# colinsongf/keyword_spotting

Hardware: AMD Instinct MI355X
Metric: mel-frames/s (real-time 10 ms-hop audio streams sustained = value/100) (higher is better)
Workload: dtype f32

## Files before the change

### keyword_spotting_amd/csrc/gru_device.h

```cpp
#pragma once
#include <type_traits>

#include "kws_internal.h"

namespace kws {

typedef float f32x4 __attribute__((ext_vector_type(4)));

__device__ __forceinline__ f32x4 mfma4(float a, float b, f32x4 c) {
    return __builtin_amdgcn_mfma_f32_16x16x4f32(a, b, c, 0, 0, 0);
}
__device__ __forceinline__ float sigmoid_f(float x) {
    return __builtin_amdgcn_rcpf(1.0f + __expf(-x));
}
__device__ __forceinline__ float tanh_f(float x) {
    return 1.0f - 2.0f * __builtin_amdgcn_rcpf(1.0f + __expf(2.0f * x));
}
#if KWS_RESIDENT_VGPR_FORM
#define KWS_MFMA_A(acc, wa, bv) acc = mfma4(wa, bv, acc)
#else
#define KWS_MFMA_A(acc, wa, bv) \
    asm volatile("v_mfma_f32_16x16x4_f32 %0, %1, %2, %0" : "+v"(acc) : "a"(wa), "v"(bv))
#endif
__device__ __forceinline__ void mfma_fence(f32x4& a, f32x4& b, f32x4& c, f32x4& d) {
    asm volatile("s_nop 15" : "+v"(a), "+v"(b), "+v"(c), "+v"(d));
}
__device__ __forceinline__ void mfma_fence(f32x4& a, f32x4& b) {
    asm volatile("s_nop 15" : "+v"(a), "+v"(b));
}
__device__ __forceinline__ void mfma_prefence(f32x4& a, f32x4& b, f32x4& c, f32x4& d) {
    asm volatile("s_nop 3" : "+v"(a), "+v"(b), "+v"(c), "+v"(d));
}
__device__ __forceinline__ void mfma_prefence(f32x4& a, f32x4& b) {
    asm volatile("s_nop 3" : "+v"(a), "+v"(b));
}
__device__ __forceinline__ f32x4 splat4(float v) { f32x4 r = {v, v, v, v}; return r; }
__device__ __forceinline__ float bitsel(unsigned m, float a, float b) {
    return __uint_as_float((__float_as_uint(a) & m) | (__float_as_uint(b) & ~m));
}
template <int I0, int I1, class F>
__device__ __forceinline__ void static_for(F&& f) {
    if constexpr (I0 < I1) {
        f(std::integral_constant<int, I0>{});
        static_for<I0 + 1, I1>(f);
    }
}
constexpr float kLog2e = 1.4426950408889634f;
typedef float f32x2 __attribute__((ext_vector_type(2)));
__device__ __forceinline__ f32x2 sigmoid2(f32x2 x) {
    const f32x2 t = x * -kLog2e;
    f32x2 e;
    e.x = __builtin_amdgcn_exp2f(t.x);
    e.y = __builtin_amdgcn_exp2f(t.y);
    const f32x2 d = e + 1.0f;
    f32x2 r;
    r.x = __builtin_amdgcn_rcpf(d.x);
    r.y = __builtin_amdgcn_rcpf(d.y);
#ifdef KWS_FAULT_INJECT
    r = r * 1.0078125f;
#endif
    return r;
}
__device__ __forceinline__ f32x2 tanh2(f32x2 x) {
    const f32x2 t = x * (2.0f * kLog2e);
    f32x2 e;
    e.x = __builtin_amdgcn_exp2f(t.x);
    e.y = __builtin_amdgcn_exp2f(t.y);
    const f32x2 d = e + 1.0f;
    f32x2 r;
    r.x = __builtin_amdgcn_rcpf(d.x);
    r.y = __builtin_amdgcn_rcpf(d.y);
    return r * -2.0f + 1.0f;
}
__device__ __forceinline__ f32x4 ld4(const float* p) { return *reinterpret_cast<const f32x4*>(p); }

__device__ __forceinline__ void lds_barrier() {
    asm volatile("s_waitcnt lgkmcnt(0)" ::: "memory");
    __builtin_amdgcn_s_barrier();
    asm volatile("" ::: "memory");
}
constexpr int kRingFrames = 16;
constexpr int xs_stride(int kcx) { return 4 * ((((kcx + 3) / 4) & 1) ? (kcx + 3) / 4 : (kcx + 3) / 4 + 1); }
struct EpilogueLds {
    float* pstage;
    float* lring;
    int* words;
    int* carry;
    int8_t* cwords;
};
constexpr size_t kEpilogueLdsBytes = (4 * 16 * 8 + kRingFrames * 16 * 8) * 4 + kRingFrames * 16 * 4 + 2 * 16 * 4;
__device__ __forceinline__ EpilogueLds epilogue_carve(char* base) {
    EpilogueLds e;
    e.pstage = reinterpret_cast<float*>(base);
    e.lring = e.pstage + 4 * 16 * 8;
    e.words = reinterpret_cast<int*>(e.lring + kRingFrames * 16 * 8);
    e.carry = e.words + kRingFrames * 16;
    e.cwords = nullptr;
    return e;
}

__device__ __forceinline__ void epilogue_fold(const EpilogueLds& e, int t, int lane) {
    if (lane < 32) {
        const int s = lane >> 1, half = lane & 1;
        f32x4 v = *reinterpret_cast<const f32x4*>(e.pstage + (0 * 16 + s) * 8 + 4 * half);
#pragma unroll
        for (int w = 1; w < 4; ++w) v += *reinterpret_cast<const f32x4*>(e.pstage + (w * 16 + s) * 8 + 4 * half);
        *reinterpret_cast<f32x4*>(e.lring + (((t & (kRingFrames - 1)) * 16 + s) * 8 + 4 * half)) = v;
    }
}

struct FoldRegs { f32x4 v[4]; };
__device__ __forceinline__ void epilogue_fold_load(const EpilogueLds& e, int lane, FoldRegs& r) {
    if (lane < 32) {
        const int s = lane >> 1, half = lane & 1;
#pragma unroll
        for (int w = 0; w < 4; ++w) r.v[w] = *reinterpret_cast<const f32x4*>(e.pstage + (w * 16 + s) * 8 + 4 * half);
    }
}
__device__ __forceinline__ void epilogue_fold_store(const EpilogueLds& e, int t, int lane, const FoldRegs& r) {
    if (lane < 32) {
        const int s = lane >> 1, half = lane & 1;
        const f32x4 v = ((r.v[0] + r.v[1]) + r.v[2]) + r.v[3];
        *reinterpret_cast<f32x4*>(e.lring + (((t & (kRingFrames - 1)) * 16 + s) * 8 + 4 * half)) = v;
    }
}

template <bool OPAQUE_LANE = false>
__device__ __forceinline__ void epilogue_flush(const GruLayerParams& p, const EpilogueLds& e, int group, int t0,
                                               int n, int w, int lane, bool final_flush) {
    if constexpr (OPAQUE_LANE) asm volatile("" : "+v"(lane));
    const int f = 4 * w + (lane & 3);
    const int s = lane >> 2;
    const int b = group * kStreamsPerGroup + s;
    const int C = p.C;
    float lg[kMaxClasses];
    {
        const f32x4* row = reinterpret_cast<const f32x4*>(e.lring + (f * 16 + s) * 8);
        const f32x4 lo = row[0], hi = row[1];
#pragma unroll
        for (int c = 0; c < 4; ++c) { lg[c] = lo[c]; lg[4 + c] = hi[c]; }
    }
    if (p.use_relu) {
#pragma unroll
        for (int c = 0; c < kMaxClasses; ++c) {
            lg[c] = fmaxf(lg[c], 0.f);
            if (p.value_clip > 0.f) lg[c] = fminf(lg[c], 20.f);
        }
    }
    float m = lg[0];
#pragma unroll
    for (int c = 1; c < kMaxClasses; ++c) m = (c < C) ? fmaxf(m, lg[c]) : m;
    float pr[kMaxClasses];
    float sum = 0.f;
#pragma unroll
    for (int c = 0; c < kMaxClasses; ++c) {
        pr[c] = (c < C) ? __expf(lg[c] - m) : 0.f;
        sum += pr[c];
    }
    const float inv = __builtin_amdgcn_rcpf(sum);
#pragma unroll
    for (int c = 0; c < kMaxClasses; ++c) pr[c] *= inv;
    int word = -1;
    float best = -1.f;
#pragma unroll
    for (int c = 1; c < kMaxClasses - 1; ++c) {
        if (c < C - 1 && pr[c] > best) { best = pr[c]; word = c - 1; }
    }
    if (!(best > p.decode_thres)) word = -1;
    e.words[f * 16 + s] = word;
    if (e.cwords != nullptr) {
        int ln = lane;
        asm volatile("" : "+v"(ln));
        const int f2 = 4 * w + (ln & 3);
        if (f2 < n) e.cwords[(ln >> 2) * kWinTailWordsStride + t0 + f2] = (int8_t)word;
    }
    const bool mine = b < p.B && f < n;
    const size_t row = (size_t)b * (p.t_stride ? p.t_stride : p.T) + (t0 + f);
    if (mine) {
        if (C == 6) {
            if (p.logits) {
                float2* o = reinterpret_cast<float2*>(p.logits + row * 6);
                o[0] = make_float2(lg[0], lg[1]); o[1] = make_float2(lg[2], lg[3]); o[2] = make_float2(lg[4], lg[5]);
            }
            if (p.softmax) {
                float2* o = reinterpret_cast<float2*>(p.softmax + row * 6);
                o[0] = make_float2(pr[0], pr[1]); o[1] = make_float2(pr[2], pr[3]); o[2] = make_float2(pr[4], pr[5]);
            }
        } else {
            if (p.logits) {
#pragma unroll
                for (int c = 0; c < kMaxClasses; ++c)
                    if (c < C) p.logits[row * C + c] = lg[c];
            }
            if (p.softmax) {
#pragma unroll
                for (int c = 0; c < kMaxClasses; ++c)
                    if (c < C) p.softmax[row * C + c] = pr[c];
            }
        }
    }
    lds_barrier();
    const int blk = (t0 / kRingFrames) & 1;
    const int prev = f == 0 ? e.carry[blk * 16 + s] : e.words[(f - 1) * 16 + s];
    const int token = (word >= 0 && word != prev) ? word + 1 : 0;
    if (f == n - 1) {
        if (!final_flush) e.carry[(blk ^ 1) * 16 + s] = word;
        else if (b < p.B && p.prev_word) p.prev_word[b] = word;
    }
    if (mine && p.tokens) p.tokens[row] = (int8_t)token;
}


}
```

### keyword_spotting_amd/csrc/gru_resident.hip

```cpp
#include <cstddef>

#include "gru_device.h"
#include "launch.h"
#include "window_device.h"

namespace kws {

#if KWS_RESIDENT_VGPR_FORM
template <class... A> __device__ __forceinline__ void resident_prefence(A&...) {}
template <class... A> __device__ __forceinline__ void resident_fence(A&...) { __builtin_amdgcn_sched_barrier(0); }
#else
template <class... A> __device__ __forceinline__ void resident_prefence(A&... a) { mfma_prefence(a...); }
template <class... A> __device__ __forceinline__ void resident_fence(A&... a) { mfma_fence(a...); }
#endif


#if KWS_RESIDENT_VGPR_FORM
constexpr int resident_kreg(int kcx, bool first, bool last, bool window) { return first ? kcx : (last && window) ? 10 : 16; }
#else
constexpr int resident_kreg(int, bool first, bool, bool) { return first ? 0 : 2; }
#endif
constexpr size_t resident_lds_bytes(int kcx, bool first, bool last, bool window) {
    size_t n = 2 * 8 * 64 * 16 + (size_t)4 * (kcx - resident_kreg(kcx, first, last, window)) * 64 * 16;
    if (!first) n += 8 * 64 * 16;
    if (last) n += kEpilogueLdsBytes;
    if (first) n += (size_t)64 * xs_stride(kcx) * 4;
    return n;
}

template <int KCX, bool FIRST, bool LAST, bool MASKED, bool WINDOW>
__device__ __forceinline__ void gru_layer_resident_body(const GruLayerParams& p) {
    static_assert(!WINDOW || (LAST && !FIRST), "the window tail belongs to the last layer of a stack");
    static_assert(!WINDOW || !MASKED, "the window tail refuses seq_len");
    constexpr int H = 128, NT = 8, KCH = 32;
    const int tid = threadIdx.x;
    const int w = __builtin_amdgcn_readfirstlane(tid >> 6);
    const int lane = tid & 63, g = lane >> 4, s = lane & 15;
    const int n_groups = (p.B + kStreamsPerGroup - 1) / kStreamsPerGroup;
    int group = blockIdx.x;
    int b_raw = group * kStreamsPerGroup + s;
    bool bvalid = b_raw < p.B;
    int b = bvalid ? b_raw : p.B - 1;
    const int T = p.T;
    const int n0 = 2 * w, n1 = 2 * w + 1;

    extern __shared__ __attribute__((aligned(16))) char smem[];
    f32x4* hbuf = reinterpret_cast<f32x4*>(smem);
    f32x4* rhbuf = hbuf + NT * 64;
    constexpr int KREG = resident_kreg(KCX, FIRST, LAST, WINDOW), KL = KCX - KREG;
    static_assert(KREG >= 0 && KREG <= KCX && 192 + 4 * KREG <= 256, "the register chunks share the 256 AGPRs with the recurrent weights");
    f32x4* wlds = rhbuf + NT * 64;
    f32x4* xsb = wlds + 4 * KL * 64;
    char* const lds_tail = reinterpret_cast<char*>(xsb + (FIRST ? 0 : NT * 64));
    static_assert(resident_lds_bytes(KCX, FIRST, LAST, WINDOW) + (WINDOW ? kWinTailWordsBytes : 0) <= 160 * 1024, "LDS per CU");
    EpilogueLds epi = epilogue_carve(lds_tail);
    if constexpr (WINDOW) epi.cwords = reinterpret_cast<int8_t*>(lds_tail + kEpilogueLdsBytes);
    const uint8_t* win_dl = reinterpret_cast<const uint8_t*>(epi.cwords) + 16 * kWinTailWordsStride;
    constexpr size_t kWinOffset = offsetof(GruLayerParams, win);
    if constexpr (WINDOW) window_tail_prepare(window_tail_params_from_kernarg(kWinOffset), const_cast<uint8_t*>(win_dl), tid);
    constexpr int kXsStride = xs_stride(KCX);
    float* xs = reinterpret_cast<float*>(lds_tail + (LAST ? kEpilogueLdsBytes : 0));

    float wgh[2][2][KCH];
    float wch[2][KCH];
    float wcx[2][KCX];
    float wgx[KREG ? KREG : 1][4];
    const f32x4* wh4 = reinterpret_cast<const f32x4*>(p.wh);
#pragma unroll
    for (int j = 0; j < 2; ++j) {
        const int n = 2 * w + j;
#pragma unroll
        for (int k4 = 0; k4 < KCH / 4; ++k4) {
            const f32x4 vr = wh4[((n * 3 + 0) * (KCH / 4) + k4) * 64 + lane];
            const f32x4 vu = wh4[((n * 3 + 1) * (KCH / 4) + k4) * 64 + lane];
            const f32x4 vc = wh4[((n * 3 + 2) * (KCH / 4) + k4) * 64 + lane];
#pragma unroll
            for (int e = 0; e < 4; ++e) {
                wgh[j][0][4 * k4 + e] = vr[e];
                wgh[j][1][4 * k4 + e] = vu[e];
                wch[j][4 * k4 + e] = vc[e];
            }
        }
    }
    if constexpr (FIRST) {
#pragma unroll
        for (int j = 0; j < 2; ++j)
#pragma unroll
            for (int kc = 0; kc < KCX; ++kc) wcx[j][kc] = p.wx[(((2 * w + j) * 3 + 2) * KCX + kc) * 64 + lane];
#pragma unroll
        for (int kc = 0; kc < KCX; ++kc) {
            f32x4 v;
            v.x = p.wx[((n0 * 3 + 0) * KCX + kc) * 64 + lane];
            v.y = p.wx[((n0 * 3 + 1) * KCX + kc) * 64 + lane];
            v.z = p.wx[((n1 * 3 + 0) * KCX + kc) * 64 + lane];
            v.w = p.wx[((n1 * 3 + 1) * KCX + kc) * 64 + lane];
            if (kc < KREG) { const int kr = kc < KREG ? kc : 0; wgx[kr][0] = v[0]; wgx[kr][1] = v[1]; wgx[kr][2] = v[2]; wgx[kr][3] = v[3]; }
            else wlds[(w * KL + kc - KREG) * 64 + lane] = v;
        }
    } else {
        const f32x4* wx4 = reinterpret_cast<const f32x4*>(p.wx);
#pragma unroll
        for (int j = 0; j < 2; ++j)
#pragma unroll
            for (int k4 = 0; k4 < KCX / 4; ++k4) {
                const f32x4 vc = wx4[(((2 * w + j) * 3 + 2) * (KCX / 4) + k4) * 64 + lane];
#pragma unroll
                for (int e = 0; e < 4; ++e) wcx[j][4 * k4 + e] = vc[e];
            }
#pragma unroll
        for (int k4 = 0; k4 < KCX / 4; ++k4) {
            const f32x4 r0 = wx4[((n0 * 3 + 0) * (KCX / 4) + k4) * 64 + lane];
            const f32x4 u0 = wx4[((n0 * 3 + 1) * (KCX / 4) + k4) * 64 + lane];
            const f32x4 r1 = wx4[((n1 * 3 + 0) * (KCX / 4) + k4) * 64 + lane];
            const f32x4 u1 = wx4[((n1 * 3 + 1) * (KCX / 4) + k4) * 64 + lane];
#pragma unroll
            for (int e = 0; e < 4; ++e) {
                const f32x4 v = {r0[e], u0[e], r1[e], u1[e]};
                const int kc = 4 * k4 + e, kr = kc < KREG ? kc : 0;
                if (kc < KREG) { wgx[kr][0] = v[0]; wgx[kr][1] = v[1]; wgx[kr][2] = v[2]; wgx[kr][3] = v[3]; }
                else wlds[(w * KL + kc - KREG) * 64 + lane] = v;
            }
        }
    }
#pragma unroll
    for (int j = 0; j < 2; ++j) {
#pragma unroll
        for (int kc = 0; kc < KCH; ++kc) {
            asm volatile("" : "+a"(wgh[j][0][kc]));
            asm volatile("" : "+a"(wgh[j][1][kc]));
            asm volatile("" : "+a"(wch[j][kc]));
        }
    }
#if KWS_RESIDENT_VGPR_FORM
    if constexpr (KREG > 0) {
#pragma unroll
        for (int kc = 0; kc < KREG; ++kc)
#pragma unroll
            for (int e = 0; e < 4; ++e) asm volatile("" : "+a"(wgx[kc][e]));
    }
#endif
    asm volatile("s_nop 7" ::: "memory");
    f32x4 bias_r[2], bias_u[2], bias_c[2];
#pragma unroll
    for (int j = 0; j < 2; ++j) {
        const int n = 2 * w + j;
        bias_r[j] = ld4(p.bias + 0 * H + n * 16 + 4 * g);
        bias_u[j] = ld4(p.bias + 1 * H + n * 16 + 4 * g);
        bias_c[j] = ld4(p.bias + 2 * H + n * 16 + 4 * g);
    }
    float wfc[2][4];
    f32x4 bfc4 = splat4(0.f);
    if (LAST) {
#pragma unroll
        for (int j = 0; j < 2; ++j)
#pragma unroll
            for (int e = 0; e < 4; ++e) wfc[j][e] = p.wfc[((2 * w + j) * 4 + e) * 64 + lane];
        if (w == 0) bfc4 = ld4(p.bfc + 4 * g);
    }

    int len_s = T;
    f32x4 hreg[2];
    const float4* xl_src = nullptr;
    const float4* xprev = nullptr;
    const float4* xg_next = nullptr;
    constexpr int XQ = KCX;
    const int xl_row = lane / XQ, xl_q = lane % XQ;
    const bool xl_active = FIRST && lane < 4 * XQ;
    auto enter_group = [&]() {
        b_raw = group * kStreamsPerGroup + s;
        bvalid = b_raw < p.B;
        b = bvalid ? b_raw : p.B - 1;
        const bool do_reset = p.reset != nullptr && p.reset[b] != 0;
        if constexpr (MASKED) len_s = p.seq_len ? p.seq_len[b] - p.t_base : T;
#pragma unroll
        for (int j = 0; j < 2; ++j) {
            const int n = 2 * w + j;
            hreg[j] = do_reset ? splat4(0.f) : ld4(p.state_in + (size_t)b * H + n * 16 + 4 * g);
            hbuf[n * 64 + lane] = hreg[j];
        }
        if (LAST && tid < 16) {
            const int bb = group * kStreamsPerGroup + tid;
            int pw = -1;
            if (bb < p.B && p.prev_word && !(p.reset && p.reset[bb])) pw = p.prev_word[bb];
            epi.carry[tid] = pw;
        }
        if constexpr (FIRST) {
            const int xl_b = min(group * kStreamsPerGroup + 4 * w + (xl_active ? xl_row : 0), p.B - 1);
            xl_src = reinterpret_cast<const float4*>(p.x_mel + (size_t)xl_b * (p.t_stride ? p.t_stride : T) * p.I) + xl_q;
        } else {
            xprev = p.x_prev + (size_t)group * T * NT * 64 + lane;
            xg_next = xprev + ((size_t)(1 < T ? 1 : 0) * NT + n0) * 64;
        }
    };

    constexpr bool kIssueAtEnd = FIRST && !LAST;
    float4 xl_inflight = make_float4(0.f, 0.f, 0.f, 0.f);
    auto coop_issue = [&](int t_req) {
        const int t = t_req < T ? t_req : T - 1;
        if (xl_active) xl_inflight = xl_src[(size_t)t * XQ];
    };
    auto coop_commit = [&]() {
        if (xl_active) {
            float* dst = xs + (4 * (4 * w + xl_row)) * kXsStride + xl_q;
            dst[0 * kXsStride] = xl_inflight.x;
            dst[1 * kXsStride] = xl_inflight.y;
            dst[2 * kXsStride] = xl_inflight.z;
            dst[3 * kXsStride] = xl_inflight.w;
        }
    };
    float xbuf0[KCX];
    auto read_xs = [&](float (&dst)[KCX]) {
        const float* row = xs + (4 * s + g) * kXsStride;
#pragma unroll
        for (int k4 = 0; k4 < KCX / 4; ++k4) {
            const f32x4 v = *reinterpret_cast<const f32x4*>(row + 4 * k4);
            dst[4 * k4 + 0] = v[0]; dst[4 * k4 + 1] = v[1]; dst[4 * k4 + 2] = v[2]; dst[4 * k4 + 3] = v[3];
        }
        if constexpr (KCX % 4 >= 2) {
            const f32x2 v = *reinterpret_cast<const f32x2*>(row + (KCX / 4) * 4);
            dst[(KCX / 4) * 4 + 0] = v[0]; dst[(KCX / 4) * 4 + 1] = v[1];
        }
        if constexpr (KCX % 2 == 1) dst[KCX - 1] = row[KCX - 1];
    };
    auto load_x_slice = [&](float (&dst)[KCX], int t_req, const int sl) {
        if constexpr (!FIRST) {
            const int t = t_req < T ? t_req : T - 1;
            const float4 v = xprev[((size_t)t * NT + sl) * 64];
            dst[4 * sl + 0] = v.x; dst[4 * sl + 1] = v.y; dst[4 * sl + 2] = v.z; dst[4 * sl + 3] = v.w;
        }
    };
    float4 xg_inflight[2];
    auto group_issue = [&](int t_req) {
        if constexpr (!FIRST) {
            xg_inflight[0] = xg_next[0];
            xg_inflight[1] = xg_next[64];
            if (t_req + 1 < T) xg_next += NT * 64;
        }
    };
    auto group_commit = [&]() {
        if constexpr (!FIRST) {
#pragma unroll
            for (int j = 0; j < 2; ++j)
                xsb[(2 * w + j) * 64 + lane] = (f32x4){xg_inflight[j].x, xg_inflight[j].y, xg_inflight[j].z, xg_inflight[j].w};
        }
    };
    auto read_x_slice = [&](float (&dst)[KCX], const int sl) {
        if constexpr (!FIRST) {
            const f32x4 v = xsb[sl * 64 + lane];
            dst[4 * sl + 0] = v[0]; dst[4 * sl + 1] = v[1]; dst[4 * sl + 2] = v[2]; dst[4 * sl + 3] = v[3];
        }
    };

    f32x4 acc_r[2], acc_u[2], acc_c[2];
    auto gates_x_part = [&](const float (&xB)[KCX], auto k0_, auto k1_, auto pin_) {
        constexpr int K0 = decltype(k0_)::value, K1 = decltype(k1_)::value;
        constexpr bool PIN = decltype(pin_)::value;
        constexpr int R0 = K0 < KREG ? KREG : K0;
        f32x4 ring[3];
        if (R0 < K1) ring[R0 % 3] = wlds[(w * KL + R0 - KREG) * 64 + lane];
        if (R0 + 1 < K1) ring[(R0 + 1) % 3] = wlds[(w * KL + R0 + 1 - KREG) * 64 + lane];
#pragma unroll
        for (int kc = K0; kc < K1; ++kc) {
            if (kc + 2 < K1 && kc + 2 >= R0 + 2) ring[(kc + 2) % 3] = wlds[(w * KL + kc + 2 - KREG) * 64 + lane];
            if (PIN) __builtin_amdgcn_sched_barrier(0);
            const int kr = kc < KREG ? kc : 0;
            const f32x4 a4 = kc < KREG ? (f32x4){wgx[kr][0], wgx[kr][1], wgx[kr][2], wgx[kr][3]} : ring[kc % 3];
            acc_r[0] = mfma4(a4.x, xB[kc], acc_r[0]);
            acc_u[0] = mfma4(a4.y, xB[kc], acc_u[0]);
            acc_r[1] = mfma4(a4.z, xB[kc], acc_r[1]);
            acc_u[1] = mfma4(a4.w, xB[kc], acc_u[1]);
            if (PIN) __builtin_amdgcn_sched_barrier(0);
        }
    };
    using pinned = std::true_type;
    constexpr int KSPLIT = KCX / 2;
    using k_lo = std::integral_constant<int, 0>;
    using k_mid = std::integral_constant<int, KSPLIT>;
    using k_hi = std::integral_constant<int, KCX>;
    auto cand_x = [&](const float (&xB)[KCX]) {
#pragma unroll
        for (int j = 0; j < 2; ++j) acc_c[j] = bias_c[j];
#pragma unroll
        for (int kc = 0; kc < KCX; ++kc) {
            acc_c[0] = mfma4(wcx[0][kc], xB[kc], acc_c[0]);
            acc_c[1] = mfma4(wcx[1][kc], xB[kc], acc_c[1]);
        }
    };

    f32x4 hb_a, hb_b;

    auto frame = [&](int t, float (&xcur)[KCX], float (&xnxt)[KCX]) {
        resident_prefence(acc_r[0], acc_u[0], acc_r[1], acc_u[1]);
#pragma unroll
        for (int nn = 0; nn < NT; ++nn) {
            const f32x4 hb = (nn & 1) ? hb_b : hb_a;
            if (nn + 2 < NT) {
                if (nn & 1) hb_b = hbuf[(nn + 2) * 64 + lane]; else hb_a = hbuf[(nn + 2) * 64 + lane];
            }
            if constexpr (FIRST) { if (!kIssueAtEnd && nn == 0) coop_issue(t + 2); }
            else { if (nn == 0) group_issue(t + 2); read_x_slice(xnxt, nn); }
            __builtin_amdgcn_sched_barrier(0);
#pragma unroll
            for (int e = 0; e < 4; ++e) {
                const int kc = 4 * nn + e;
                const float hv = hb[e];
                KWS_MFMA_A(acc_r[0], wgh[0][0][kc], hv);
                KWS_MFMA_A(acc_u[0], wgh[0][1][kc], hv);
                KWS_MFMA_A(acc_r[1], wgh[1][0][kc], hv);
                KWS_MFMA_A(acc_u[1], wgh[1][1][kc], hv);
            }
        }
        resident_fence(acc_r[0], acc_u[0], acc_r[1], acc_u[1]);
        if constexpr (FIRST) read_xs(xcur);
        f32x4 u[2];
#pragma unroll
        for (int j = 0; j < 2; ++j) {
            const f32x2 r_lo = sigmoid2((f32x2){acc_r[j][0], acc_r[j][1]});
            const f32x2 r_hi = sigmoid2((f32x2){acc_r[j][2], acc_r[j][3]});
            const f32x2 rh_lo = r_lo * (f32x2){hreg[j][0], hreg[j][1]};
            const f32x2 rh_hi = r_hi * (f32x2){hreg[j][2], hreg[j][3]};
            rhbuf[(2 * w + j) * 64 + lane] = (f32x4){rh_lo.x, rh_lo.y, rh_hi.x, rh_hi.y};
        }
#pragma unroll
        for (int j = 0; j < 2; ++j) {
            const f32x2 u_lo = sigmoid2((f32x2){acc_u[j][0], acc_u[j][1]});
            const f32x2 u_hi = sigmoid2((f32x2){acc_u[j][2], acc_u[j][3]});
            u[j] = (f32x4){u_lo.x, u_lo.y, u_hi.x, u_hi.y};
        }
#pragma unroll
        for (int j = 0; j < 2; ++j) { acc_r[j] = bias_r[j]; acc_u[j] = bias_u[j]; }
        __builtin_amdgcn_sched_barrier(0);
        gates_x_part(xcur, k_lo{}, k_mid{}, pinned{});
        lds_barrier();
        hb_a = rhbuf[0 * 64 + lane];
        hb_b = rhbuf[1 * 64 + lane];
        group_commit();
        gates_x_part(xcur, k_mid{}, k_hi{}, pinned{});

        resident_prefence(acc_c[0], acc_c[1]);
#pragma unroll
        for (int nn = 0; nn < NT; ++nn) {
            const f32x4 rb = (nn & 1) ? hb_b : hb_a;
            if (nn + 2 < NT) {
                if (nn & 1) hb_b = rhbuf[(nn + 2) * 64 + lane]; else hb_a = rhbuf[(nn + 2) * 64 + lane];
            }
            __builtin_amdgcn_sched_barrier(0);
#pragma unroll
            for (int e = 0; e < 4; ++e) {
                const int kc = 4 * nn + e;
                const float rv = rb[e];
                KWS_MFMA_A(acc_c[0], wch[0][kc], rv);
                KWS_MFMA_A(acc_c[1], wch[1][kc], rv);
            }
        }
        resident_fence(acc_c[0], acc_c[1]);
        const unsigned live = !MASKED || t < len_s ? 0xffffffffu : 0u;
        f32x4 hout[2];
#pragma unroll
        for (int j = 0; j < 2; ++j) {
#pragma unroll
            for (int h2 = 0; h2 < 2; ++h2) {
                const f32x2 c = tanh2((f32x2){acc_c[j][2 * h2], acc_c[j][2 * h2 + 1]});
                const f32x2 uu = {u[j][2 * h2], u[j][2 * h2 + 1]};
                const f32x2 hh = {hreg[j][2 * h2], hreg[j][2 * h2 + 1]};
                const f32x2 hn = __builtin_elementwise_fma(uu, hh, (1.0f - uu) * c);
                if constexpr (!MASKED) {
                    hreg[j][2 * h2] = hn.x;
                    hreg[j][2 * h2 + 1] = hn.y;
                    continue;
                }
                hreg[j][2 * h2] = bitsel(live, hn.x, hh.x);
                hreg[j][2 * h2 + 1] = bitsel(live, hn.y, hh.y);
                if (LAST) {
                    hout[j][2 * h2] = bitsel(live, hn.x, 0.f);
                    hout[j][2 * h2 + 1] = bitsel(live, hn.y, 0.f);
                }
            }
        }
#pragma unroll
        for (int j = 0; j < 2; ++j) acc_c[j] = bias_c[j];
        constexpr int NCX = 2 * KCX;
        constexpr int NPOST = NCX >= 32 ? 16 : 8;
        constexpr int NPRE = NCX - NPOST;
        auto cand_x_mfma = [&](auto mc) {
            constexpr int m = decltype(mc)::value, kc = m / 2;
            if constexpr (m % 2 == 0) acc_c[0] = mfma4(wcx[0][kc], xcur[kc], acc_c[0]);
            else acc_c[1] = mfma4(wcx[1][kc], xcur[kc], acc_c[1]);
        };
        if constexpr (FIRST) {
            coop_commit();
            if constexpr (kIssueAtEnd) coop_issue(t + 3);
        }
#pragma unroll
        for (int j = 0; j < 2; ++j) {
            hbuf[(2 * w + j) * 64 + lane] = hreg[j];
            if (!LAST) {
                const f32x4 o = hreg[j];
                p.h_out[((size_t)group * T + t) * NT * 64 + (2 * w + j) * 64 + lane] =
                    make_float4(o[0], o[1], o[2], o[3]);
            }
        }
        if (LAST) {
            f32x4 accf = bfc4;
#pragma unroll
            for (int j = 0; j < 2; ++j)
#pragma unroll
                for (int e = 0; e < 4; ++e) accf = mfma4(wfc[j][e], MASKED ? hout[j][e] : hreg[j][e], accf);
            if (g < 2) *reinterpret_cast<f32x4*>(epi.pstage + (w * 16 + s) * 8 + 4 * g) = accf;
        }
        __builtin_amdgcn_sched_barrier(0);
        static_for<0, NPRE>(cand_x_mfma);
        __builtin_amdgcn_sched_barrier(0);
        lds_barrier();
        hb_a = hbuf[0 * 64 + lane];
        hb_b = hbuf[1 * 64 + lane];
        FoldRegs fold;
        const bool folder = LAST && w == (t & 3);
        if (folder) epilogue_fold_load(epi, lane, fold);
        __builtin_amdgcn_sched_barrier(0);
        static_for<NPRE, NCX>(cand_x_mfma);
        __builtin_amdgcn_sched_barrier(0);
        if (LAST) {
            if (folder) epilogue_fold_store(epi, t, lane, fold);
            if (((t + 1) & (kRingFrames - 1)) == 0 || t == T - 1) {
                const int t0 = t & ~(kRingFrames - 1);
                lds_barrier();
                epilogue_flush(p, epi, group, t0, t - t0 + 1, w, lane, t == T - 1);
            }
        }
    };

    for (; group < n_groups; group += gridDim.x) {
    enter_group();
    if constexpr (!FIRST) {
        if (T > 0) {
            group_issue(1);
#pragma unroll
            for (int sl = 0; sl < NT; ++sl) load_x_slice(xbuf0, 0, sl);
            group_commit();
        }
    }
    __syncthreads();
    if (T > 0) {
        if constexpr (FIRST) {
            coop_issue(0);
            coop_commit();
            __syncthreads();
            read_xs(xbuf0);
            coop_issue(1);
        }
#pragma unroll
        for (int j = 0; j < 2; ++j) { acc_r[j] = bias_r[j]; acc_u[j] = bias_u[j]; }
        gates_x_part(xbuf0, k_lo{}, k_hi{}, pinned{});
        hb_a = hbuf[0 * 64 + lane];
        hb_b = hbuf[1 * 64 + lane];
        cand_x(xbuf0);
        if constexpr (FIRST) {
            __syncthreads();
            coop_commit();
            if constexpr (kIssueAtEnd) coop_issue(2);
            __syncthreads();
        }
    }
    for (int t = 0; t < T; ++t) frame(t, xbuf0, xbuf0);

    if (bvalid) {
#pragma unroll
        for (int j = 0; j < 2; ++j)
            *reinterpret_cast<f32x4*>(p.state_out + (size_t)b * H + (2 * w + j) * 16 + 4 * g) = hreg[j];
    }
    __syncthreads();
    if constexpr (WINDOW) {
        const WindowTail win = window_tail_params_from_kernarg(kWinOffset);
        WindowTailRegs<2> wreq;
        window_tail_request<2>(win, p.B, group * kStreamsPerGroup, tid, wreq);
        window_tail<2>(win, p.B, group * kStreamsPerGroup, T, epi.cwords, kWinTailWordsStride, win_dl, reinterpret_cast<char*>(hbuf), tid, wreq);
        __syncthreads();
    }
    }
}

template <int KCX, bool FIRST, bool LAST, bool WINDOW = false>
__global__ void __launch_bounds__(256) __attribute__((amdgpu_waves_per_eu(1, 1)))
gru_layer_resident(const GruLayerParams p) { gru_layer_resident_body<KCX, FIRST, LAST, false, WINDOW>(p); }
template <int KCX, bool FIRST, bool LAST>
__global__ void __launch_bounds__(256) __attribute__((amdgpu_waves_per_eu(1, 1)))
gru_layer_resident_masked(const GruLayerParams p) { gru_layer_resident_body<KCX, FIRST, LAST, true, false>(p); }
template <int KCX, bool FIRST, bool LAST, bool MASKED>
inline constexpr auto resident_kernel = MASKED ? &gru_layer_resident_masked<KCX, FIRST, LAST> : &gru_layer_resident<KCX, FIRST, LAST, false>;

int gru_resident_kcx(int in_dim, bool first) { return first ? (in_dim + 3) / 4 : 32; }

bool gru_resident_supported(int hidden, int in_dim, bool first) {
    if (hidden != 128) return false;
    if (!first) return in_dim == 128;
    return in_dim == 32 || in_dim == 40 || in_dim == 48 || in_dim == 60 || in_dim == 64;
}

bool gru_resident_takes_window(bool first, bool last) { return last && !first; }

hipError_t launch_gru_layer_resident(const GruLayerParams& p, bool first, bool last, hipStream_t st) {
    const bool window = p.win.tab != nullptr;
    const size_t lds = resident_lds_bytes(p.KCX, first, last, window);
    const dim3 grid(persistent_grid(p.B));
    if (window) {
        if (!gru_resident_takes_window(first, last) || p.seq_len) return hipErrorInvalidValue;
        return launch_lds<gru_layer_resident<32, false, true, true>>(grid, dim3(256), lds + kWinTailWordsBytes, st, p);
    }
    return with_bool(p.seq_len != nullptr, [&](auto ma) {
        return with_bool(last, [&](auto la) {
            if (!first) return launch_lds<resident_kernel<32, false, la(), ma()>>(grid, dim3(256), lds, st, p);
            return with_int<8, 10, 12, 15, 16>(p.KCX, [&](auto kcx) {
                return launch_lds<resident_kernel<kcx(), true, la(), ma()>>(grid, dim3(256), lds, st, p);
            });
        });
    });
}

}
```

Before: 409.7 million.

## Store per-wave FC partials in LDS ring and fold them at flush time

```diff
diff --git a/keyword_spotting_amd/csrc/gru_device.h b/keyword_spotting_amd/csrc/gru_device.h
--- a/keyword_spotting_amd/csrc/gru_device.h
+++ b/keyword_spotting_amd/csrc/gru_device.h
@@ -109,22 +109,6 @@
     }
 }
 
-struct FoldRegs { f32x4 v[4]; };
-__device__ __forceinline__ void epilogue_fold_load(const EpilogueLds& e, int lane, FoldRegs& r) {
-    if (lane < 32) {
-        const int s = lane >> 1, half = lane & 1;
-#pragma unroll
-        for (int w = 0; w < 4; ++w) r.v[w] = *reinterpret_cast<const f32x4*>(e.pstage + (w * 16 + s) * 8 + 4 * half);
-    }
-}
-__device__ __forceinline__ void epilogue_fold_store(const EpilogueLds& e, int t, int lane, const FoldRegs& r) {
-    if (lane < 32) {
-        const int s = lane >> 1, half = lane & 1;
-        const f32x4 v = ((r.v[0] + r.v[1]) + r.v[2]) + r.v[3];
-        *reinterpret_cast<f32x4*>(e.lring + (((t & (kRingFrames - 1)) * 16 + s) * 8 + 4 * half)) = v;
-    }
-}
-
 template <bool OPAQUE_LANE = false>
 __device__ __forceinline__ void epilogue_flush(const GruLayerParams& p, const EpilogueLds& e, int group, int t0,
                                                int n, int w, int lane, bool final_flush) {
@@ -210,5 +194,88 @@
     if (mine && p.tokens) p.tokens[row] = (int8_t)token;
 }
 
-
-}
+constexpr int kPartialSlotFloats = 4 * 16 * 8 + 4;
+constexpr size_t kPartialRingLdsBytes = (size_t)kRingFrames * kPartialSlotFloats * 4;
+__device__ __forceinline__ float* partial_slot(float* ring, int t) { return ring + (t & (kRingFrames - 1)) * kPartialSlotFloats; }
+
+__device__ __forceinline__ void epilogue_flush_partials(const GruLayerParams& p, const float* ring, int8_t* cwords, int group,
+                                                        int t0, int n, int w, int lane, bool final_flush, int& carry) {
+    asm volatile("" : "+v"(lane));
+    const int f = lane & 15;
+    const int s = 4 * w + (lane >> 4);
+    const int b = group * kStreamsPerGroup + s;
+    const int C = p.C;
+    float lg[kMaxClasses];
+    {
+        const f32x4* row = reinterpret_cast<const f32x4*>(ring + f * kPartialSlotFloats + s * 8);
+        f32x4 lo = row[0], hi = row[1];
+#pragma unroll
+        for (int k = 1; k < 4; ++k) { lo += row[k * 32]; hi += row[k * 32 + 1]; }
+#pragma unroll
+        for (int c = 0; c < 4; ++c) { lg[c] = lo[c]; lg[4 + c] = hi[c]; }
+    }
+    if (p.use_relu) {
+#pragma unroll
+        for (int c = 0; c < kMaxClasses; ++c) {
+            lg[c] = fmaxf(lg[c], 0.f);
+            if (p.value_clip > 0.f) lg[c] = fminf(lg[c], 20.f);
+        }
+    }
+    float m = lg[0];
+#pragma unroll
+    for (int c = 1; c < kMaxClasses; ++c) m = (c < C) ? fmaxf(m, lg[c]) : m;
+    float pr[kMaxClasses];
+    float sum = 0.f;
+#pragma unroll
+    for (int c = 0; c < kMaxClasses; ++c) {
+        pr[c] = (c < C) ? __expf(lg[c] - m) : 0.f;
+        sum += pr[c];
+    }
+    const float inv = __builtin_amdgcn_rcpf(sum);
+#pragma unroll
+    for (int c = 0; c < kMaxClasses; ++c) pr[c] *= inv;
+    int word = -1;
+    float best = -1.f;
+#pragma unroll
+    for (int c = 1; c < kMaxClasses - 1; ++c) {
+        if (c < C - 1 && pr[c] > best) { best = pr[c]; word = c - 1; }
+    }
+    if (!(best > p.decode_thres)) word = -1;
+    if (cwords != nullptr && f < n) cwords[s * kWinTailWordsStride + t0 + f] = (int8_t)word;
+    const bool mine = b < p.B && f < n;
+    const size_t row = (size_t)b * (p.t_stride ? p.t_stride : p.T) + (t0 + f);
+    if (mine) {
+        if (C == 6) {
+            if (p.logits) {
+                float2* o = reinterpret_cast<float2*>(p.logits + row * 6);
+                o[0] = make_float2(lg[0], lg[1]); o[1] = make_float2(lg[2], lg[3]); o[2] = make_float2(lg[4], lg[5]);
+            }
+            if (p.softmax) {
+                float2* o = reinterpret_cast<float2*>(p.softmax + row * 6);
+                o[0] = make_float2(pr[0], pr[1]); o[1] = make_float2(pr[2], pr[3]); o[2] = make_float2(pr[4], pr[5]);
+            }
+        } else {
+            if (p.logits) {
+#pragma unroll
+                for (int c = 0; c < kMaxClasses; ++c)
+                    if (c < C) p.logits[row * C + c] = lg[c];
+            }
+            if (p.softmax) {
+#pragma unroll
+                for (int c = 0; c < kMaxClasses; ++c)
+                    if (c < C) p.softmax[row * C + c] = pr[c];
+            }
+        }
+    }
+    const int prev = __builtin_amdgcn_update_dpp(carry, word, 0x111, 0xf, 0xf, false);
+    const int token = (word >= 0 && word != prev) ? word + 1 : 0;
+    if (mine && p.tokens) p.tokens[row] = (int8_t)token;
+    if (final_flush) {
+        if (f == n - 1 && b < p.B && p.prev_word) p.prev_word[b] = word;
+    } else {
+        carry = __builtin_amdgcn_ds_bpermute(((lane & 48) + n - 1) << 2, word);
+    }
+}
+
+
+}
diff --git a/keyword_spotting_amd/csrc/gru_resident.hip b/keyword_spotting_amd/csrc/gru_resident.hip
--- a/keyword_spotting_amd/csrc/gru_resident.hip
+++ b/keyword_spotting_amd/csrc/gru_resident.hip
@@ -23,7 +23,7 @@
 constexpr size_t resident_lds_bytes(int kcx, bool first, bool last, bool window) {
     size_t n = 2 * 8 * 64 * 16 + (size_t)4 * (kcx - resident_kreg(kcx, first, last, window)) * 64 * 16;
     if (!first) n += 8 * 64 * 16;
-    if (last) n += kEpilogueLdsBytes;
+    if (last) n += kPartialRingLdsBytes;
     if (first) n += (size_t)64 * xs_stride(kcx) * 4;
     return n;
 }
@@ -53,13 +53,13 @@
     f32x4* xsb = wlds + 4 * KL * 64;
     char* const lds_tail = reinterpret_cast<char*>(xsb + (FIRST ? 0 : NT * 64));
     static_assert(resident_lds_bytes(KCX, FIRST, LAST, WINDOW) + (WINDOW ? kWinTailWordsBytes : 0) <= 160 * 1024, "LDS per CU");
-    EpilogueLds epi = epilogue_carve(lds_tail);
-    if constexpr (WINDOW) epi.cwords = reinterpret_cast<int8_t*>(lds_tail + kEpilogueLdsBytes);
-    const uint8_t* win_dl = reinterpret_cast<const uint8_t*>(epi.cwords) + 16 * kWinTailWordsStride;
+    float* const pring = reinterpret_cast<float*>(lds_tail);
+    int8_t* const cwords = WINDOW ? reinterpret_cast<int8_t*>(lds_tail + kPartialRingLdsBytes) : nullptr;
+    const uint8_t* win_dl = reinterpret_cast<const uint8_t*>(cwords) + 16 * kWinTailWordsStride;
     constexpr size_t kWinOffset = offsetof(GruLayerParams, win);
     if constexpr (WINDOW) window_tail_prepare(window_tail_params_from_kernarg(kWinOffset), const_cast<uint8_t*>(win_dl), tid);
     constexpr int kXsStride = xs_stride(KCX);
-    float* xs = reinterpret_cast<float*>(lds_tail + (LAST ? kEpilogueLdsBytes : 0));
+    float* xs = reinterpret_cast<float*>(lds_tail + (LAST ? kPartialRingLdsBytes : 0));
 
     float wgh[2][2][KCH];
     float wch[2][KCH];
@@ -159,6 +159,7 @@
     }
 
     int len_s = T;
+    int carry = -1;
     f32x4 hreg[2];
     const float4* xl_src = nullptr;
     const float4* xprev = nullptr;
@@ -178,11 +179,10 @@
             hreg[j] = do_reset ? splat4(0.f) : ld4(p.state_in + (size_t)b * H + n * 16 + 4 * g);
             hbuf[n * 64 + lane] = hreg[j];
         }
-        if (LAST && tid < 16) {
-            const int bb = group * kStreamsPerGroup + tid;
-            int pw = -1;
-            if (bb < p.B && p.prev_word && !(p.reset && p.reset[bb])) pw = p.prev_word[bb];
-            epi.carry[tid] = pw;
+        if (LAST) {
+            const int bb = group * kStreamsPerGroup + 4 * w + (lane >> 4);
+            carry = -1;
+            if (bb < p.B && p.prev_word && !(p.reset && p.reset[bb])) carry = p.prev_word[bb];
         }
         if constexpr (FIRST) {
             const int xl_b = min(group * kStreamsPerGroup + 4 * w + (xl_active ? xl_row : 0), p.B - 1);
@@ -400,13 +400,14 @@
                     make_float4(o[0], o[1], o[2], o[3]);
             }
         }
-        if (LAST) {
+        if constexpr (LAST) {
+            __builtin_amdgcn_sched_barrier(0);
             f32x4 accf = bfc4;
 #pragma unroll
             for (int j = 0; j < 2; ++j)
 #pragma unroll
                 for (int e = 0; e < 4; ++e) accf = mfma4(wfc[j][e], MASKED ? hout[j][e] : hreg[j][e], accf);
-            if (g < 2) *reinterpret_cast<f32x4*>(epi.pstage + (w * 16 + s) * 8 + 4 * g) = accf;
+            if (g < 2) *reinterpret_cast<f32x4*>(partial_slot(pring, t) + (w * 16 + s) * 8 + 4 * g) = accf;
         }
         __builtin_amdgcn_sched_barrier(0);
         static_for<0, NPRE>(cand_x_mfma);
@@ -414,18 +415,13 @@
         lds_barrier();
         hb_a = hbuf[0 * 64 + lane];
         hb_b = hbuf[1 * 64 + lane];
-        FoldRegs fold;
-        const bool folder = LAST && w == (t & 3);
-        if (folder) epilogue_fold_load(epi, lane, fold);
         __builtin_amdgcn_sched_barrier(0);
         static_for<NPRE, NCX>(cand_x_mfma);
         __builtin_amdgcn_sched_barrier(0);
-        if (LAST) {
-            if (folder) epilogue_fold_store(epi, t, lane, fold);
+        if constexpr (LAST) {
             if (((t + 1) & (kRingFrames - 1)) == 0 || t == T - 1) {
                 const int t0 = t & ~(kRingFrames - 1);
-                lds_barrier();
-                epilogue_flush(p, epi, group, t0, t - t0 + 1, w, lane, t == T - 1);
+                epilogue_flush_partials(p, pring, cwords, group, t0, t - t0 + 1, w, lane, t == T - 1, carry);
             }
         }
     };
@@ -474,7 +470,7 @@
         const WindowTail win = window_tail_params_from_kernarg(kWinOffset);
         WindowTailRegs<2> wreq;
         window_tail_request<2>(win, p.B, group * kStreamsPerGroup, tid, wreq);
-        window_tail<2>(win, p.B, group * kStreamsPerGroup, T, epi.cwords, kWinTailWordsStride, win_dl, reinterpret_cast<char*>(hbuf), tid, wreq);
+        window_tail<2>(win, p.B, group * kStreamsPerGroup, T, cwords, kWinTailWordsStride, win_dl, reinterpret_cast<char*>(hbuf), tid, wreq);
         __syncthreads();
     }
     }
```

Measured after the change: 414.1 million (median of 6 runs). 1.01x the previous value.
